# PJLab-ADG/OpenPCSeg

Hardware: AMD Instinct MI355X
Metric: LiDAR frames/sec training MinkUNet-34 SemanticKITTI (higher is better)
Workload: dtype f32; 1 GPU; MinkUNet-34 cr1.0 train step, 12 x 120k-pt synthetic SemanticKITTI scans/GPU, fp32; global_batch=12, voxels_per_gpu_batch=1158864, parallelism=dp1, wgrad=fp32

## Files before the change

include/pcseg_hip.h:

```cpp
#ifndef PCSEG_HIP_H_
#define PCSEG_HIP_H_

#include <stddef.h>
#include <stdint.h>

#ifdef __cplusplus
extern "C" {
#endif

#define PCS_OK 0
#define PCS_EINVAL (-1)
#define PCS_EWORKSPACE (-2)
#define PCS_ELAUNCH (-3)
#define PCS_EUNSUPPORTED (-4)

#define PCS_ABI_VERSION 12

int pcs_abi_version(void);
const char *pcs_last_error(void);

int pcs_hash(const int32_t *coords, int64_t n, int64_t *out, void *stream);

int pcs_kernel_hash(const int32_t *coords, int64_t n, const int32_t *offsets, int32_t K,
                    int64_t *out, void *stream);

int64_t pcs_hashtable_capacity(int64_t n);
size_t pcs_hashtable_bytes(int64_t capacity);
int pcs_hashtable_build(const int64_t *keys, int64_t n, void *table, int64_t capacity,
                        void *stream);
int pcs_hashtable_query(const void *table, int64_t capacity, const int64_t *queries,
                        int64_t n1, int64_t *out, void *stream);

int pcs_count(const int32_t *idx, int64_t n, int32_t *out, int64_t s, void *stream);

int pcs_voxelize_fwd_f32(const float *feats, const int32_t *idx, const int32_t *counts,
                         int64_t n, int64_t m, int32_t c, float *out, void *stream);
size_t pcs_index_csr_ws_bytes(int64_t n, int64_t m);
int pcs_index_csr_i32(const int32_t *index, int64_t n, int64_t m, int64_t *order, int64_t *rowptr, void *ws,
                      size_t ws_bytes, void *stream);
int pcs_voxelize_fwd_csr_f32(const float *feats, const int64_t *order, const int64_t *rowptr,
                             const int32_t *counts, int64_t m, int32_t c, float *out, void *stream);
int pcs_voxelize_bwd_f32(const float *gout, const int32_t *idx, const int32_t *counts,
                         int64_t n, int32_t c, float *gin, void *stream);

int pcs_devoxelize_fwd_f32(const float *feat, const int32_t *idx8, const float *w8, int64_t n,
                           int32_t c, float *out, void *stream);
int pcs_devoxelize_bwd_f32(const float *gout, const int32_t *idx8, const float *w8, int64_t n,
                           int64_t m, int32_t c, float *gfeat, void *stream);

int pcs_corner_map_f32(const float *coords, int32_t coord_ld, int64_t n, int32_t stride, const void *table,
                       int64_t capacity, int32_t *idx8, float *w8, void *stream);

int pcs_devoxelize_bwd_csr_f32(const float *gout, const int64_t *order, const int64_t *rowptr,
                               const float *w8, int64_t m, int32_t c, float *gfeat, void *stream);

int pcs_ti_weights_f32(const float *coords, int32_t coord_ld, const int64_t *idx_query,
                       int64_t n, float scale, float *w, void *stream);

int pcs_downsample_pack(const int32_t *coords, int64_t n, const int32_t *sample_stride3,
                        int32_t mode, const int32_t *offsets, int32_t K,
                        const int32_t *coords_min3, int64_t *keys, int32_t *err, void *stream);
int pcs_downsample_unpack(const int64_t *keys, int64_t m, int32_t *coords, void *stream);
size_t pcs_sort_unique_ws_bytes(int64_t n);
int pcs_sort_unique_i64(const int64_t *keys, int64_t n, int64_t *out, int64_t *info, const int32_t *err_flag, void *ws,
                        size_t ws_bytes, void *stream);

size_t pcs_rulebook_ws_bytes(int64_t nq, int32_t K);
int pcs_rulebook_probe(const int32_t *qcoords, int64_t nq, const int32_t *offsets, int32_t K,
                       const void *table, int64_t capacity, int32_t *results,
                       int64_t *nbsizes, void *ws, size_t ws_bytes, int32_t symmetric, void *stream);
int pcs_rulebook_fill(const int32_t *results, int64_t nq, int32_t K, const void *ws,
                      int32_t *pairs, int32_t *koff, void *stream);
int pcs_rulebook_tile_segments(const int32_t *pairs, const int32_t *koff, int32_t K,
                               int64_t n_dst, int32_t tile_rows, int32_t dst_col,
                               int32_t *seg, void *stream);
int pcs_rulebook_tile_order(const int32_t *seg, int32_t K, int64_t ntiles, int32_t *order, void *stream);

const char *pcs_conv_kernel_revision(void);
int32_t pcs_conv_tile_rows(int32_t cin, int32_t cout);
int32_t pcs_conv_pick_tile_rows(int64_t n_dst, int64_t n_pairs, int32_t K, int32_t cin, int32_t cout);
int32_t pcs_conv_pick_tile_rows_dt(int64_t n_dst, int64_t n_pairs, int32_t K, int32_t cin, int32_t cout,
                                   int32_t dtype);
int32_t pcs_conv_emits_bn_partials(int32_t cin, int32_t cout, int32_t K, int32_t tile_rows, int32_t dtype);
int32_t pcs_conv_uses_tile_order(int32_t cin, int32_t cout, int32_t K, int32_t dtype);
int pcs_conv_gather_gemm_f32(const float *src, int64_t n_src, int32_t cin, const float *W,
                             int32_t K, int32_t cout, const int32_t *pairs, int32_t src_col,
                             const int32_t *seg, int32_t tile_rows, int64_t n_dst,
                             const float *bias, float *dst, double *bn_partial, const int32_t *tile_order,
                             void *stream);
typedef struct pcs_conv_epilogue {
  const void *addend;
  float act_slope;
  int32_t reserved;
} pcs_conv_epilogue;
int pcs_conv_gather_gemm_f32_ex(const float *src, int64_t n_src, int32_t cin, const float *W,
                                int32_t K, int32_t cout, const int32_t *pairs, int32_t src_col,
                                const int32_t *seg, int32_t tile_rows, int64_t n_dst,
                                const float *bias, const pcs_conv_epilogue *ep, float *dst, double *bn_partial,
                                const int32_t *tile_order, void *stream);
int32_t pcs_conv_supports_epilogue(int32_t cin, int32_t cout, int32_t K, int32_t dtype);

int pcs_transpose_kab_f32(const float *src, int32_t K, int32_t A, int32_t B, float *dst, void *stream);

size_t pcs_conv_wgrad_ws_bytes(const int32_t *koff_host, int32_t K, int32_t ca, int32_t cb);
int pcs_conv_wgrad_f32(const float *fa, int32_t ca, const float *fb, int32_t cb,
                       const int32_t *pairs, int32_t a_col, const int32_t *koff_dev,
                       const int32_t *koff_host, int32_t K, float *gW, void *ws,
                       size_t ws_bytes, void *stream);

int pcs_scatter_max_fwd_f32(const float *src, const int64_t *order, const int64_t *rowptr, int64_t m,
                            int32_t c, float *out, int32_t *arg, void *stream);
int pcs_scatter_max_bwd_f32(const float *gout, const int32_t *arg, int64_t m, int64_t n, int32_t c,
                            float *gsrc, void *stream);

int pcs_map_count(const int32_t *pxpy, int64_t n, int32_t B, int32_t H, int32_t W, int32_t *out,
                  void *stream);
int pcs_denselize_fwd_f32(const float *feat, const int32_t *count_map, const int32_t *pxpy, int64_t n,
                          int32_t B, int32_t C, int32_t H, int32_t W, float *out, void *stream);
int pcs_denselize_fwd_csr_f32(const float *feat, const int64_t *order, const int64_t *rowptr,
                              const int32_t *count_map, int32_t B, int32_t C, int32_t H, int32_t W,
                              float *out, void *stream);
int pcs_denselize_bwd_csr_f32(const float *gout, const int64_t *order, const int64_t *rowptr,
                              const int32_t *count_map, int64_t n, int32_t B, int32_t C, int32_t H, int32_t W,
                              float *gfeat, void *stream);
int pcs_denselize_bwd_f32(const float *gout, const int32_t *count_map, const int32_t *pxpy, int64_t n,
                          int32_t B, int32_t C, int32_t H, int32_t W, float *gfeat, void *stream);

int pcs_range_sample_fwd_f32(const float *img, const float *pxpy, int64_t n, int32_t B, int32_t C, int32_t H, int32_t W,
                             float *out, void *stream);
int pcs_range_sample_corners(const float *pxpy, int64_t n, int32_t B, int32_t H, int32_t W, int64_t *keys, float *wts,
                             void *stream);
int pcs_range_sample_bwd_csr_f32(const float *gout, const int64_t *order, const int64_t *rowptr, const float *wts,
                                 int32_t B, int32_t C, int32_t H, int32_t W, float *gimg, void *stream);

int32_t pcs_bn_num_partials(void);
int pcs_bn_stats_f32(const float *x, int64_t n, int32_t c, float *partial_ws, double *sums, void *stream);
int pcs_bn_reduce_partials(const double *partial, int64_t nrows, int32_t c, int64_t n, double *sums, void *stream);
int pcs_bn_reduce_partials_finalize(const double *partial, int64_t nrows, int32_t c, int64_t n, double eps, double momentum,
                                    float *running_mean, float *running_var, double *sums, double *stat, void *stream);
int pcs_bn_finalize_f32(const double *sums, double count, const double *count_dev, int32_t c, double eps,
                        double momentum, float *running_mean, float *running_var, double *stat, void *stream);
int pcs_bn_apply_f32(const float *x, const float *res, const double *stat, const float *w, const float *b,
                     int64_t n, int32_t c, int32_t relu, float *y, uint32_t *mask, int64_t ldy, const float *tail,
                     int32_t ctail, void *stream);
int pcs_bn_bwd_stats_f32(const float *dy, const float *x, const float *y, const uint32_t *mask, const double *stat,
                         int64_t n, int32_t c, int32_t relu, float *partial_ws, double *sums2, int64_t sums2_doubles,
                         int64_t lddy, void *stream);
int pcs_bn_bwd_apply_f32(const float *dy, const float *x, const float *y, const uint32_t *mask, const double *stat,
                         const double *sums2, double count, const double *count_dev, const float *w, int64_t n,
                         int32_t c, int32_t relu, float *dx, float *dres, int64_t lddy, void *stream);
int pcs_bn_stats_h(const void *x, int64_t n, int32_t c, int32_t dtype, float *partial_ws, double *sums, void *stream);
int pcs_bn_apply_h(const void *x, const void *res, const double *stat, const float *w, const float *b, int64_t n,
                   int32_t c, int32_t relu, int32_t dtype, void *y, uint32_t *mask, int64_t ldy, const void *tail,
                   int32_t ctail, void *stream);
int pcs_bn_bwd_stats_h(const void *dy, const void *x, const void *y, const uint32_t *mask, const double *stat, int64_t n,
                       int32_t c, int32_t relu, int32_t dtype, float *partial_ws, double *sums2, int64_t sums2_doubles,
                       int64_t lddy, void *stream);
int pcs_bn_bwd_apply_h(const void *dy, const void *x, const void *y, const uint32_t *mask, const double *stat,
                       const double *sums2, double count, const double *count_dev, const float *w, int64_t n,
                       int32_t c, int32_t relu, int32_t dtype, void *dx, void *dres, int64_t lddy, void *stream);
int pcs_bn_bwd_apply_act(const void *dy, const void *x, const void *y, const uint32_t *mask, const double *stat,
                         const double *sums2, double count, const double *count_dev, const float *w, int64_t n, int32_t c,
                         int32_t relu, int32_t dtype, float in_slope, void *dx, void *dres, int64_t lddy, void *stream);

int pcs_quantize_floor(const void *points, int32_t is_float, int64_t n, int32_t row_stride,
                       const double *voxel_size3, int32_t *coords, int32_t *bbox, void *stream);
int pcs_quantize_keys(const int32_t *coords, int64_t n, const int32_t *bbox, int64_t *keys, void *stream);
int pcs_quantize_frame_keys(const int32_t *coords, const int64_t *frames, int64_t n, const int32_t *bbox, int64_t *keys, void *stream);
int pcs_quantize_flags(const int64_t *sorted_keys, int64_t n, int32_t *flags, void *stream);
int pcs_quantize_emit(const int32_t *flags, const int64_t *rank, const int64_t *perm, const int32_t *coords,
                      int64_t n, int32_t *vox, int64_t *index, int64_t *inverse, void *stream);

int pcs_unique_emit(const int32_t *flags, const int64_t *rank, const int64_t *perm, const int64_t *sorted_keys,
                    int64_t n, int64_t *uniq, int64_t *inverse, int64_t *rowptr, void *stream);

int pcs_conv_x3_applies(int32_t cin, int32_t cout, int32_t K);
int32_t pcs_conv_x3_column_tiles(int32_t cout);
int32_t pcs_conv_x3_emits_bn_partials(int32_t cin, int32_t cout, int32_t K, int32_t tile_rows);
size_t pcs_conv_prepared_weights_x3_bytes(int32_t K, int32_t ccon, int32_t ccols);
int pcs_conv_prepare_weights_x3(const float *W, int32_t K, int32_t A, int32_t B, int32_t transpose, void *Wp, void *stream);
int pcs_conv_gather_gemm_f32_bf16x3(const float *src, int64_t n_src, int32_t cin, const void *Wp, int32_t K, int32_t cout,
                                    const int32_t *pairs, int32_t src_col, const int32_t *seg, int32_t tile_rows,
                                    int64_t n_dst, const float *bias, float *dst, double *bn_partial,
// ... 54 lines not shown
```

openpcseg_amd/csrc/conv.hip:

```cpp
#include <math.h>

#include "conv_half.h"

using namespace pcs;

namespace pcs {
bool conv6h_applies(int cin, int cout, int K);
bool conv6h_is_chunked(int cin, int cout);
int conv6h_mode();
}

namespace {

int device_cus() {
  static int cus = 0;
  if (!cus) {
    int dev = 0, n = 0;
    if (hipGetDevice(&dev) == hipSuccess &&
        hipDeviceGetAttribute(&n, hipDeviceAttributeMultiprocessorCount, dev) == hipSuccess && n > 0) cus = n;
    else cus = 256;
  }
  return cus;
}

__global__ void __launch_bounds__(256) transpose_kab_kernel(const float *__restrict__ src, int A, int B,
                                                            float *__restrict__ dst) {
  __shared__ float tile[32][33];
  const int k = blockIdx.z, a0 = blockIdx.y * 32, b0 = blockIdx.x * 32;
  const int tx = threadIdx.x & 31, ty = threadIdx.x >> 5;
  const float *s = src + (int64_t)k * A * B;
  float *d = dst + (int64_t)k * A * B;
#pragma unroll
  for (int r = ty; r < 32; r += 8)
    if (a0 + r < A && b0 + tx < B) tile[r][tx] = s[(int64_t)(a0 + r) * B + b0 + tx];
  __syncthreads();
#pragma unroll
  for (int r = ty; r < 32; r += 8)
    if (b0 + r < B && a0 + tx < A) d[(int64_t)(b0 + r) * A + a0 + tx] = tile[tx][r];
}

}

extern "C" int pcs_transpose_kab_f32(const float *src, int32_t K, int32_t A, int32_t B, float *dst, void *stream) {
  if (K <= 0 || A <= 0 || B <= 0 || K > 65535 || !src || !dst) { set_error("pcs_transpose_kab_f32: bad args"); return PCS_EINVAL; }
  hipLaunchKernelGGL(transpose_kab_kernel, dim3((unsigned)ceil_div(B, 32), (unsigned)ceil_div(A, 32), (unsigned)K), dim3(256),
                     0, as_stream(stream), src, A, B, dst);
  return check_launch("pcs_transpose_kab_f32");
}

extern "C" const char *pcs_conv_kernel_revision(void) { return "r6.1"; }

extern "C" int32_t pcs_conv_tile_rows(int32_t cin, int32_t cout) {
  (void)cin;
  (void)cout;
  return 128;
}

namespace {
double launch_cost(int64_t n_dst, int T, int64_t ncol, double ppr, int K) {
  const double per_cu = (double)(ceil_div(n_dst, T) * ncol) / (double)device_cus();
  const double rounds = 0.5 * (ceil(per_cu) + per_cu);
  return rounds * (T * ppr + 8.0 * K);
}
}

extern "C" int32_t pcs_conv_pick_tile_rows_dt(int64_t n_dst, int64_t n_pairs, int32_t K, int32_t cin, int32_t cout,
                                              int32_t dtype) {
  static const int fixed = getenv("PCS_CONV_TILE") ? atoi(getenv("PCS_CONV_TILE")) : 0;
  if (n_dst <= 0 || K <= 0 || cin <= 0 || cout <= 0) return 128;
  if (!(dtype == 0 ? conv5_applies(cin, cout, K) : convh_applies(cin, cout, K))) return 128;
  if (fixed > 0) return fixed;
  const double ppr = (double)n_pairs / (double)n_dst;
  const int nctt = conv_nctt(cout);
  if (dtype != 0) {
    if (cin >= 256 && cout >= 256) {
      if (conv6h_mode() && conv6h_applies(cin, cout, K) && conv6h_is_chunked(cin, cout) && (cin > 256 || cout > 256 || n_dst <= 65536))
        return 144;
      const int64_t ncol = ceil_div(cout, 16 * nctt);
      return launch_cost(n_dst, 288, ncol, ppr, K) <= launch_cost(n_dst, 224, ncol, ppr, K) ? 288 : 224;
    }
    const int64_t ncol = ceil_div(cout, 16 * nctt);
    const int tmax = nctt == 6 ? 192 : 144;
    int best = tmax;
    double best_cost = launch_cost(n_dst, tmax, ncol, ppr, K);
    for (int T = tmax - 16; T >= tmax - 48; T -= 16) {
      const double c = launch_cost(n_dst, T, ncol, ppr, K);
      if (c < best_cost * 0.97) { best = T; best_cost = c; }
    }
    return best;
  }
  if (conv5_nctt(cout, 192) <= 4) {
    const int64_t ncol = ceil_div(cout, 16 * conv5_nctt(cout, 192));
    int best = 224;
    double best_cost = 0;
    for (int T = 192; T <= 288; T += 32) {
      const double c = launch_cost(n_dst, T, ncol, ppr, K);
      if (best_cost == 0 || c < best_cost) { best = T; best_cost = c; }
    }
    return best;
  }
  const int64_t ncol = ceil_div(cout, 16 * nctt);
  const int64_t slots = (int64_t)device_cus() * 2;
  if (ceil_div(n_dst, 128) * ncol >= 8 * slots && ppr < 6.5) {
    int T = 384;
    while (T > 128 && conv5_lds_est(T, nctt) > kMaxDynLds) T -= 32;
    if (T >= 192) return T;
  }
  int best = 128;
  double best_cost = launch_cost(n_dst, 128, ncol, ppr, K) * 0.97;
  for (int T = 80; T <= 192; T += 16) {
    if (T == 128) continue;
    if (2 * conv5_lds_est(T, nctt) > 160 * 1024) continue;
    const double c = launch_cost(n_dst, T, ncol, ppr, K);
    if (c < best_cost) { best = T; best_cost = c; }
  }
  return best;
}

extern "C" int32_t pcs_conv_pick_tile_rows(int64_t n_dst, int64_t n_pairs, int32_t K, int32_t cin, int32_t cout) {
  return pcs_conv_pick_tile_rows_dt(n_dst, n_pairs, K, cin, cout, 0);
}

extern "C" int32_t pcs_conv_emits_bn_partials(int32_t cin, int32_t cout, int32_t K, int32_t tile_rows, int32_t dtype) {
  if (cin <= 0 || cout <= 0 || K <= 0 || K > 32 || (cin % 4) || (cout % 4) || tile_rows < 16) return 0;
  int nctt = conv_nctt(cout), nt = 256;
  if (dtype == 0) {
    if (conv5_applies(cin, cout, K)) {
      nctt = conv5_nctt(cout, tile_rows);
      nt = 2 * conv5_lds_est(tile_rows, nctt) > 160 * 1024 ? 512 : 256;
    } else if (tile_rows != 64 && tile_rows != 128) {
      return 0;
    }
  } else {
// ... 69 lines not shown
```

openpcseg_amd/csrc/conv_common.h:

```cpp
#pragma once
#include <stdlib.h>

#include <type_traits>

#include "pcs_common.h"

#ifndef PCS_TRACE
#define PCS_TRACE 0
#endif
#ifndef PCS_ABLATE5
#define PCS_ABLATE5 0
#endif
#ifndef PCS_ABLATEH
#define PCS_ABLATEH 0
#endif
#ifndef PCS_ALIAS
#define PCS_ALIAS 0
#endif
#if PCS_TRACE
#define PCS_T(...) __VA_ARGS__
#else
#define PCS_T(...)
#endif

namespace pcs {

typedef float f32x4 __attribute__((ext_vector_type(4)));

struct ConvArgs {
  const float *src;
  const float *W;
  const float *bias;
  float *dst;
  const int32_t *pairs;
  const int32_t *seg;
  int64_t n_dst;
  int64_t ntiles;
  int cin, cout, K, src_col, ncoltiles, tile_rows;
  double *stats;
  const int32_t *order;
  const float *addend = nullptr;
  float act_slope = 1.f;
};

struct Bf16 {};
struct Fp16 {};
struct Fp32 {};
__device__ __forceinline__ float h2f(Bf16, uint16_t h) { return __uint_as_float((uint32_t)h << 16); }
__device__ __forceinline__ float h2f(Fp16, uint16_t h) { return (float)__builtin_bit_cast(_Float16, h); }
__device__ __forceinline__ uint16_t f2h(Bf16, float f) {
  uint32_t u = __float_as_uint(f);
  if ((u & 0x7FFFFFFFu) > 0x7F800000u) return (uint16_t)((u >> 16) | 0x40u);
  u += 0x7FFFu + ((u >> 16) & 1u);
  return (uint16_t)(u >> 16);
}
__device__ __forceinline__ uint16_t f2h(Fp16, float f) {
  const _Float16 h = (_Float16)f;
  return __builtin_bit_cast(uint16_t, h);
}

constexpr size_t kMaxDynLds = 160 * 1024 - 256;
constexpr int kConvSinkRows = 1;
inline size_t conv5_lds_est(int tile_rows, int nctt) { return (size_t)((tile_rows + kConvSinkRows) * (16 * nctt + 4)) * 4 + 1024; }

inline int conv_nctt(int cout) {
  int nctt = (cout + 15) / 16;
  if (nctt <= 8) {
    if (nctt == 5) nctt = 6;
    if (nctt == 7) nctt = 8;
    return nctt;
  }
  int best = 8, best_pad = ((cout + 127) / 128) * 128 - cout;
  for (int n = 6; n >= 4; n -= 2) {
    const int pad = ((cout + 16 * n - 1) / (16 * n)) * 16 * n - cout;
    if (pad < best_pad) { best = n; best_pad = pad; }
  }
  return best;
}
inline int conv5_nctt(int cout, int tile_rows) {
  if (cout >= 128 && cout % 64 == 0 && tile_rows >= 176) return 4;
  if (cout >= 192 && tile_rows >= 192) return 4;
  return conv_nctt(cout);
}
inline bool conv5_applies(int cin, int cout, int K) {
  return cin % 4 == 0 && cin >= 32 && cout % 4 == 0 && K <= 32 && conv_nctt(cout) % 2 == 0;
}

inline bool convh_applies(int cin, int cout, int K) {
  return cin % 8 == 0 && cin >= 32 && cout % 4 == 0 && K <= 32 && conv_nctt(cout) % 2 == 0;
}

template <int CT, int NT, typename Store>
__device__ __forceinline__ void conv_tile_epilogue(float *acc_l, int ACS, int rows, int n0, int cout, const float *bias,
                                                   double *stats, int tid, Store store) {
  constexpr int Q = CT / 4, NRG = NT / Q;
  const int q = tid % Q, rg = tid / Q, cq = 4 * q;
  const bool on = rg < NRG && n0 + cq < cout;
  float4 b = make_float4(0.f, 0.f, 0.f, 0.f), piv = b, s0 = b, s1 = b;
  if (on) {
    if (bias) b = *reinterpret_cast<const float4 *>(bias + n0 + cq);
    if (stats) {
      piv = *reinterpret_cast<const float4 *>(acc_l + cq);
      piv.x += b.x; piv.y += b.y; piv.z += b.z; piv.w += b.w;
    }
    for (int r = rg; r < rows; r += NRG) {
      float4 v = *reinterpret_cast<const float4 *>(acc_l + r * ACS + cq);
      v.x += b.x; v.y += b.y; v.z += b.z; v.w += b.w;
      const float4 sv = store(r, cq, v);
      if (stats) {
        const float dx = sv.x - piv.x, dy = sv.y - piv.y, dz = sv.z - piv.z, dw = sv.w - piv.w;
        s0.x += dx; s0.y += dy; s0.z += dz; s0.w += dw;
        s1.x += dx * dx; s1.y += dy * dy; s1.z += dz * dz; s1.w += dw * dw;
      }
    }
  }
  if (stats) {
    __syncthreads();
    if (on) {
      *reinterpret_cast<float4 *>(acc_l + (2 * rg) * ACS + cq) = s0;
      *reinterpret_cast<float4 *>(acc_l + (2 * rg + 1) * ACS + cq) = s1;
      if (rg == 0) *reinterpret_cast<float4 *>(acc_l + (2 * NRG) * ACS + cq) = piv;
    }
    __syncthreads();
    if (tid < CT && n0 + tid < cout) {
      double t0 = 0.0, t1 = 0.0;
      for (int h = 0; h < NRG; ++h) { t0 += (double)acc_l[(2 * h) * ACS + tid]; t1 += (double)acc_l[(2 * h + 1) * ACS + tid]; }
      const double p = (double)acc_l[(2 * NRG) * ACS + tid], dn = (double)rows;
      stats[n0 + tid] = t0 + dn * p;
      stats[cout + n0 + tid] = t1 + 2.0 * p * t0 + dn * p * p;
    }
  }
}
inline bool conv_stats_fit(int tile_rows, int ct, int nt) { return tile_rows + 1 >= 2 * (nt / (ct / 4)) + 1; }

int launch_conv_block(ConvArgs a, bool vec, hipStream_t st);
int launch_conv_wave4(ConvArgs a, hipStream_t st);
int launch_conv_wave5(ConvArgs a, hipStream_t st);

}
```

openpcseg_amd/csrc/conv_wave5.hip:

```cpp
#include "conv_common.h"

using namespace pcs;

namespace {

#if PCS_TRACE
__device__ long long *g_conv_trace;
constexpr int kTraceBlocks = 8192;
#endif

template <int NCTT, int NW_, int R_>
struct Conv5Cfg {
  static constexpr int NW = NW_;
  static constexpr int R = R_;
  static constexpr int NT = 64 * NW;
  static constexpr int CT = 16 * NCTT;
  static constexpr int ACS = CT + 4;
  static constexpr int N4 = NCTT / 4;
  static constexpr int N2 = (NCTT % 4) / 2;
  static constexpr int N1 = NCTT % 2;
  static constexpr int NWL = N4 + N2 + N1;
  static constexpr int SINK = kConvSinkRows;
  static constexpr size_t lds_bytes(int T) { return (size_t)((T + SINK) * ACS) * 4 + 5 * 33 * 4 + 16; }
};

template <int NCTT, int NW, int MINW, int R, bool TAIL>
__global__ void __launch_bounds__(64 * NW, MINW) conv_os5_kernel(ConvArgs a) {
  using C = Conv5Cfg<NCTT, NW, R>;
  const int T = a.tile_rows;
  PCS_T(const long long tr_entry = wall_clock64(); long long tr_loop = 0, tr_ticket = 0, tr_commit = 0; int tr_groups = 0;)
  extern __shared__ __attribute__((aligned(16))) char smem[];
  float *acc_l = reinterpret_cast<float *>(smem);
  int *kl_k = reinterpret_cast<int *>(acc_l + (T + C::SINK) * C::ACS);
  int *kl_s = kl_k + 32;
  int *kl_m = kl_s + 32;
  int *kl_g = kl_m + 32;
  int *kl_h = kl_g + 33;
  int *commit = kl_h + 33;
  const unsigned commit_lds = (unsigned)(size_t)(__attribute__((address_space(3))) int *)commit;
  const unsigned acc_lds = (unsigned)(size_t)(__attribute__((address_space(3))) float *)acc_l;
  __shared__ int nk_s;

  const int tid = threadIdx.x, lane = tid & 63, wid = __builtin_amdgcn_readfirstlane(tid >> 6);
  const int g = lane >> 4, l15 = lane & 15;
  unsigned bid = blockIdx.x;
  if (!a.order) {
    const unsigned nb = gridDim.x, q = nb >> 3, r = nb & 7, xcd = bid & 7, idx = bid >> 3;
    bid = (xcd < r ? xcd * (q + 1) : r * (q + 1) + (xcd - r) * q) + idx;
  }
  int64_t slot = bid / a.ncoltiles;
  int ctile = bid % a.ncoltiles;
  if (a.order) {
    const unsigned xcd = bid & 7, idx = bid >> 3;
    slot = (int64_t)(idx / a.ncoltiles) * 8 + xcd;
    ctile = idx % a.ncoltiles;
    if (slot >= a.ntiles) return;
  }
  const int64_t tile = a.order ? (int64_t)a.order[slot] : slot;
  const int n0 = ctile * C::CT;
  const int64_t row0 = tile * T;
  const int64_t nt1 = a.ntiles + 1;

  if (wid == 0) {
    const int k = lane;
    int s0 = 0, m = 0;
    if (k < a.K) {
      s0 = a.seg[(int64_t)k * nt1 + tile];
      m = a.seg[(int64_t)k * nt1 + tile + 1] - s0;
    }
    const unsigned long long mask = __ballot(m > 0);
    const int nrb = (m + 15) >> 4;
    const int nfull = nrb / R, npart = (nrb % R) ? 1 : 0;
    int incl = nfull | (npart << 16);
    for (int o = 1; o < 64; o <<= 1) {
      const int t = __shfl_up(incl, o, 64);
      if (lane >= o) incl += t;
    }
    if (m > 0) {
      const int pos = __popcll(mask & ((1ULL << lane) - 1ULL));
      kl_k[pos] = k; kl_s[pos] = s0; kl_m[pos] = m;
      kl_g[pos] = (incl & 0xFFFF) - nfull; kl_h[pos] = (incl >> 16) - npart;
    }
    const int total = __shfl(incl, 63, 64);
    if (lane == 0) {
      const int nkk = __popcll(mask);
      nk_s = nkk; kl_g[nkk] = total & 0xFFFF; kl_h[nkk] = total >> 16; *commit = 0;
    }
  }
  {
    float4 *z = reinterpret_cast<float4 *>(acc_l);
    const int n4 = (T + C::SINK) * (C::ACS / 4);
    for (int i = tid; i < n4; i += C::NT) z[i] = make_float4(0.f, 0.f, 0.f, 0.f);
  }
  __syncthreads();
  const int nk = __builtin_amdgcn_readfirstlane(nk_s);
  const int total_full = nk > 0 ? __builtin_amdgcn_readfirstlane(kl_g[nk]) : 0;
  const int total_grp = nk > 0 ? total_full + __builtin_amdgcn_readfirstlane(kl_h[nk]) : 0;

  const int cin4 = a.cin - 4;
  const int nb16 = TAIL ? (a.cin + 15) >> 4 : a.cin >> 4;
  const int cinp = nb16 * 16;
  int col4[C::N4 > 0 ? C::N4 : 1];
#pragma unroll
  for (int q = 0; q < C::N4; ++q) {
    const int c = 64 * q + 4 * l15;
    col4[q] = (n0 + c + 4 <= a.cout) ? c : 0;
  }
  const int c2 = 64 * C::N4 + 2 * l15;
  const int col2 = (n0 + c2 + 2 <= a.cout) ? c2 : 0;
  const int c1 = 64 * C::N4 + 32 * C::N2 + l15;
  const int col1 = (n0 + c1 < a.cout) ? c1 : 0;

  struct Frag {
    float4 a[R];
    float4 b4[4][C::N4 > 0 ? C::N4 : 1];
    float2 b2[4];
    float b1[4];
  };
  struct Ctx {
    const float *srow0[R];
    const float *Wk;
    int dloc[R];
    int nr;
    unsigned vmask;
  };
  auto load_frag = [&](Frag &f, const Ctx &cx, int c0, bool in_loop = false) {
    int ca = c0 + 4 * g;
    if (TAIL) ca = ca < cin4 ? ca : cin4;
    (void)in_loop;
#if PCS_ABLATE5 == 3
    if (in_loop) return;
#endif
#if PCS_ABLATE5 != 6
#pragma unroll
    for (int r = 0; r < R; ++r) f.a[r] = *reinterpret_cast<const float4 *>(cx.srow0[r] + ca);
#else
    if (!in_loop) for (int r = 0; r < R; ++r) f.a[r] = *reinterpret_cast<const float4 *>(cx.srow0[r] + ca);
#endif
#if PCS_ABLATE5 == 5
    if (in_loop) return;
#endif
// ... 164 lines not shown
#pragma unroll
    for (int r = 0; r < R; ++r)
#pragma unroll
      for (int j = 0; j < 4; ++j) {
        dq[r][j] = acc_lds + 4u * (unsigned)doff[r][j] + 16u * l15;
        dp[r][j] = acc_lds + 4u * (unsigned)doff[r][j] + 256u * C::N4 + (C::N2 ? 8u : 4u) * l15;
        asm volatile("" : "+v"(dq[r][j]), "+v"(dp[r][j]));
      }
    if (lane == 0) {
      while (__hip_atomic_load(commit, __ATOMIC_RELAXED, __HIP_MEMORY_SCOPE_WORKGROUP) != grp)
        __builtin_amdgcn_s_sleep(1);
    }
    __builtin_amdgcn_fence(__ATOMIC_ACQUIRE, "workgroup", "local");
    __builtin_amdgcn_s_setprio(3);
    PCS_T(const long long tr_c = wall_clock64();)
    {
      typedef float v2f __attribute__((ext_vector_type(2)));
      typedef __attribute__((address_space(3))) const f32x4 lds_cf4;
      typedef __attribute__((address_space(3))) const v2f lds_cf2;
      typedef __attribute__((address_space(3))) const float lds_cf1;
      typedef __attribute__((address_space(3))) f32x4 lds_f4;
      typedef __attribute__((address_space(3))) v2f lds_f2;
      typedef __attribute__((address_space(3))) float lds_f1;
      constexpr int RB = (NCTT <= 6) ? NRC : 1;
#pragma unroll
      for (int r0 = 0; r0 < NRC; r0 += RB) {
        f32x4 v4[RB][4][C::N4 > 0 ? C::N4 : 1];
        v2f v2[RB][4];
        float v1[RB][4];
#pragma unroll
        for (int rr = 0; rr < RB; ++rr)
#pragma unroll
          for (int j = 0; j < 4; ++j) {
            const int r = r0 + rr;
#pragma unroll
            for (int q = 0; q < C::N4; ++q) v4[rr][j][q] = *(lds_cf4 *)(size_t)(dq[r][j] + 256u * q);
            if (C::N2) v2[rr][j] = *(lds_cf2 *)(size_t)dp[r][j];
            if (C::N1) v1[rr][j] = *(lds_cf1 *)(size_t)(dp[r][j] + 128u * C::N2);
          }
        asm volatile("" ::: "memory");
#pragma unroll
        for (int rr = 0; rr < RB; ++rr)
#pragma unroll
          for (int j = 0; j < 4; ++j) {
            const int r = r0 + rr;
#pragma unroll
            for (int q = 0; q < C::N4; ++q) {
              v4[rr][j][q].x += acc[r][4 * q + 0][j]; v4[rr][j][q].y += acc[r][4 * q + 1][j];
              v4[rr][j][q].z += acc[r][4 * q + 2][j]; v4[rr][j][q].w += acc[r][4 * q + 3][j];
            }
            if (C::N2) { v2[rr][j].x += acc[r][4 * C::N4 + 0][j]; v2[rr][j].y += acc[r][4 * C::N4 + 1][j]; }
            if (C::N1) v1[rr][j] += acc[r][NCTT - 1][j];
          }
        asm volatile("" ::: "memory");
#pragma unroll
        for (int rr = 0; rr < RB; ++rr)
#pragma unroll
          for (int j = 0; j < 4; ++j) {
            const int r = r0 + rr;
#pragma unroll
            for (int q = 0; q < C::N4; ++q) *(lds_f4 *)(size_t)(dq[r][j] + 256u * q) = v4[rr][j][q];
            if (C::N2) *(lds_f2 *)(size_t)dp[r][j] = v2[rr][j];
            if (C::N1) *(lds_f1 *)(size_t)(dp[r][j] + 128u * C::N2) = v1[rr][j];
          }
        asm volatile("" ::: "memory");
      }
    }
    if (lane == 0) asm volatile("ds_write_b32 %0, %1" ::"v"(commit_lds), "v"(grp + 1) : "memory");
    __builtin_amdgcn_s_setprio(0);
    PCS_T(const long long tr_d = wall_clock64(); tr_loop += tr_b - tr_a; tr_ticket += tr_c - tr_b; tr_commit += tr_d - tr_c; ++tr_groups;)
    cur = nxt;
    i = in;
  };
  {
    int grp = wid;
    for (; grp < total_full; grp += C::NW) run_group(grp, std::integral_constant<int, R>{});
    for (; grp < total_grp; grp += C::NW) run_group(grp, std::integral_constant<int, 1>{});
  }
  PCS_T(const long long tr_end = wall_clock64();)
  __syncthreads();
  const int rows = (int)((a.n_dst - row0) < (int64_t)T ? (a.n_dst - row0) : (int64_t)T);
  float *drow = a.dst + row0 * a.cout + n0;
  const int ldd = a.cout;
  conv_tile_epilogue<C::CT, C::NT>(acc_l, C::ACS, rows, n0, a.cout, a.bias, a.stats ? a.stats + tile * 2 * a.cout : nullptr, tid,
                                   [&](int r, int cq, const float4 &v0) {
                                     float4 v = v0;
                                     if (a.addend) {
                                       const float4 ad = *reinterpret_cast<const float4 *>(a.addend + (row0 + r) * (int64_t)ldd + n0 + cq);
                                       v.x += ad.x; v.y += ad.y; v.z += ad.z; v.w += ad.w;
                                     }
                                     if (a.act_slope != 1.f) {
                                       v.x = v.x < 0.f ? v.x * a.act_slope : v.x; v.y = v.y < 0.f ? v.y * a.act_slope : v.y;
                                       v.z = v.z < 0.f ? v.z * a.act_slope : v.z; v.w = v.w < 0.f ? v.w * a.act_slope : v.w;
                                     }
                                     *reinterpret_cast<float4 *>(drow + (int64_t)r * ldd + cq) = v;
                                     return v;
                                   });
#if PCS_TRACE
  if (lane == 0 && blockIdx.x < kTraceBlocks && g_conv_trace) {
    long long *t = g_conv_trace + ((int64_t)blockIdx.x * 8 + wid) * 8;
    t[0] = tr_entry; t[1] = tr_start; t[2] = tr_end; t[3] = tr_loop; t[4] = tr_ticket; t[5] = tr_commit;
    t[6] = tr_groups; t[7] = wall_clock64();
  }
#endif
}

#if PCS_TRACE
long long *g_trace_host_ptr = nullptr;
void trace_prepare(hipStream_t st) {
  if (!g_trace_host_ptr) {
    (void)hipMalloc(&g_trace_host_ptr, (size_t)kTraceBlocks * 64 * sizeof(long long));
    (void)hipMemcpyToSymbol(HIP_SYMBOL(g_conv_trace), &g_trace_host_ptr, sizeof(g_trace_host_ptr));
  }
  (void)hipMemsetAsync(g_trace_host_ptr, 0, (size_t)kTraceBlocks * 64 * sizeof(long long), st);
}
#endif

template <int NCTT, int NW, int MINW, int R, bool TAIL>
int launch_conv5(const ConvArgs &a, hipStream_t st) {
  using C = Conv5Cfg<NCTT, NW, R>;
  const int64_t nblocks = a.order ? ceil_div(a.ntiles, 8) * 8 * a.ncoltiles : a.ntiles * a.ncoltiles;
  if (nblocks <= 0) return PCS_OK;
  if (nblocks > 0x7FFFFFFF) { set_error("pcs_conv: grid too large"); return PCS_EUNSUPPORTED; }
  auto kern = conv_os5_kernel<NCTT, NW, MINW, R, TAIL>;
  const size_t lds = C::lds_bytes(a.tile_rows);
  if (lds > kMaxDynLds) { set_error("pcs_conv: tile_rows too large for this column tile"); return PCS_EUNSUPPORTED; }
  static bool attr_set = false;
  if (!attr_set) {
    (void)hipFuncSetAttribute(reinterpret_cast<const void *>(kern),
                              hipFuncAttributeMaxDynamicSharedMemorySize, (int)kMaxDynLds);
    attr_set = true;
  }
  PCS_T(trace_prepare(st);)
  static const int dbg = getenv("PCS_CONV_DEBUG") ? atoi(getenv("PCS_CONV_DEBUG")) : 0;
  static long long dbg_last = -1;
  const long long dbg_key = ((long long)a.tile_rows << 32) ^ ((long long)a.cin << 16) ^ a.cout;
  if (dbg && dbg_key != dbg_last) {
    dbg_last = dbg_key;
    int nb = 0;
    (void)hipOccupancyMaxActiveBlocksPerMultiprocessor(&nb, reinterpret_cast<const void *>(kern), C::NT, lds);
    fprintf(stderr, "[pcs_conv] wave5<%d,%d,%d,%d%s> T=%d cin=%d cout=%d grid=%lld lds=%zu resident WG/CU=%d (waves/SIMD=%d)\n", NCTT, NW,
            MINW, R, TAIL ? ",tail" : "", a.tile_rows, a.cin, a.cout, (long long)nblocks, lds, nb, nb * NW / 4);
  }
  hipLaunchKernelGGL(kern, dim3((unsigned)nblocks), dim3(C::NT), lds, st, a);
  return check_launch("pcs_conv_gather_gemm_f32(wave5)");
}

}

#if PCS_TRACE
extern "C" int pcs_debug_conv_trace(long long *host_out) {
  if (!g_trace_host_ptr || !host_out) return PCS_EINVAL;
  if (hipDeviceSynchronize() != hipSuccess) return PCS_ELAUNCH;
  return hipMemcpy(host_out, g_trace_host_ptr, (size_t)kTraceBlocks * 64 * sizeof(long long), hipMemcpyDeviceToHost) == hipSuccess ? PCS_OK : PCS_ELAUNCH;
}
#endif

int pcs::launch_conv_wave5(ConvArgs a, hipStream_t st) {
  int nctt = conv5_nctt(a.cout, a.tile_rows);
  static const int force_nctt = getenv("PCS_CONV_NCTT") ? atoi(getenv("PCS_CONV_NCTT")) : 0;
  static const int force_nw = getenv("PCS_CONV_NW") ? atoi(getenv("PCS_CONV_NW")) : 0;
  if (force_nctt && nctt > force_nctt) nctt = force_nctt;
  a.ncoltiles = (int)ceil_div(a.cout, 16 * nctt);
  const bool nw8 = force_nw ? force_nw == 8 : 2 * conv5_lds_est(a.tile_rows, nctt) > 160 * 1024;
  const bool tail = (a.cin % 32) != 0;
#define PCS_CONV5_CASE(N)                                                                           \
  case N:                                                                                           \
    if (nw8) return tail ? launch_conv5<N, 8, 2, 2, true>(a, st) : launch_conv5<N, 8, 2, 2, false>(a, st);  \
    return tail ? launch_conv5<N, 4, 2, 2, true>(a, st) : launch_conv5<N, 4, 2, 2, false>(a, st);
  switch (nctt) {
    PCS_CONV5_CASE(2)
    PCS_CONV5_CASE(4)
    PCS_CONV5_CASE(6)
    PCS_CONV5_CASE(8)
  }
#undef PCS_CONV5_CASE
  set_error("pcs_conv_gather_gemm_f32: unreachable");
  return PCS_EINVAL;
}
```

openpcseg_amd/native.py:

```python
import ctypes
import os
from ctypes import c_char_p, c_double, c_float, c_int32, c_int64, c_size_t, c_void_p

import torch

_LIB_PATH = os.environ.get("PCS_LIB_PATH") or os.path.join(os.path.dirname(os.path.abspath(__file__)), "lib",
                                                          "libpcseg_hip.so")

_P = c_void_p
SIGNATURES = {
    "pcs_abi_version": (c_int32, []),
    "pcs_last_error": (c_char_p, []),
    "pcs_hash": (c_int32, [_P, c_int64, _P, _P]),
    "pcs_kernel_hash": (c_int32, [_P, c_int64, _P, c_int32, _P, _P]),
    "pcs_hashtable_capacity": (c_int64, [c_int64]),
    "pcs_hashtable_bytes": (c_size_t, [c_int64]),
    "pcs_hashtable_build": (c_int32, [_P, c_int64, _P, c_int64, _P]),
    "pcs_hashtable_query": (c_int32, [_P, c_int64, _P, c_int64, _P, _P]),
    "pcs_count": (c_int32, [_P, c_int64, _P, c_int64, _P]),
    "pcs_voxelize_fwd_f32": (c_int32, [_P, _P, _P, c_int64, c_int64, c_int32, _P, _P]),
    "pcs_voxelize_fwd_csr_f32": (c_int32, [_P, _P, _P, _P, c_int64, c_int32, _P, _P]),
    "pcs_voxelize_bwd_f32": (c_int32, [_P, _P, _P, c_int64, c_int32, _P, _P]),
    "pcs_devoxelize_fwd_f32": (c_int32, [_P, _P, _P, c_int64, c_int32, _P, _P]),
    "pcs_devoxelize_bwd_f32": (c_int32, [_P, _P, _P, c_int64, c_int64, c_int32, _P, _P]),
    "pcs_devoxelize_bwd_csr_f32": (c_int32, [_P, _P, _P, _P, c_int64, c_int32, _P, _P]),
    "pcs_corner_map_f32": (c_int32, [_P, c_int32, c_int64, c_int32, _P, c_int64, _P, _P, _P]),
    "pcs_ti_weights_f32": (c_int32, [_P, c_int32, _P, c_int64, c_float, _P, _P]),
    "pcs_downsample_pack": (c_int32, [_P, c_int64, _P, c_int32, _P, c_int32, _P, _P, _P, _P]),
    "pcs_downsample_unpack": (c_int32, [_P, c_int64, _P, _P]),
    "pcs_index_csr_ws_bytes": (c_size_t, [c_int64, c_int64]),
    "pcs_index_csr_i32": (c_int32, [_P, c_int64, c_int64, _P, _P, _P, c_size_t, _P]),
    "pcs_sort_unique_ws_bytes": (c_size_t, [c_int64]),
    "pcs_sort_unique_i64": (c_int32, [_P, c_int64, _P, _P, _P, _P, c_size_t, _P]),
    "pcs_rulebook_ws_bytes": (c_size_t, [c_int64, c_int32]),
    "pcs_rulebook_probe": (c_int32, [_P, c_int64, _P, c_int32, _P, c_int64, _P, _P, _P, c_size_t, c_int32, _P]),
    "pcs_rulebook_fill": (c_int32, [_P, c_int64, c_int32, _P, _P, _P, _P]),
    "pcs_rulebook_tile_segments": (c_int32, [_P, _P, c_int32, c_int64, c_int32, c_int32, _P, _P]),
    "pcs_rulebook_tile_order": (c_int32, [_P, c_int32, c_int64, _P, _P]),
    "pcs_conv_kernel_revision": (c_char_p, []),
    "pcs_conv_tile_rows": (c_int32, [c_int32, c_int32]),
    "pcs_conv_pick_tile_rows": (c_int32, [c_int64, c_int64, c_int32, c_int32, c_int32]),
    "pcs_conv_pick_tile_rows_dt": (c_int32, [c_int64, c_int64, c_int32, c_int32, c_int32, c_int32]),
    "pcs_conv_emits_bn_partials": (c_int32, [c_int32, c_int32, c_int32, c_int32, c_int32]),
    "pcs_conv_uses_tile_order": (c_int32, [c_int32, c_int32, c_int32, c_int32]),
    "pcs_conv_gather_gemm_f32": (c_int32, [_P, c_int64, c_int32, _P, c_int32, c_int32, _P, c_int32,
                                           _P, c_int32, c_int64, _P, _P, _P, _P, _P]),
    "pcs_conv_gather_gemm_f32_ex": (c_int32, [_P, c_int64, c_int32, _P, c_int32, c_int32, _P, c_int32,
                                              _P, c_int32, c_int64, _P, _P, _P, _P, _P, _P]),
    "pcs_conv_supports_epilogue": (c_int32, [c_int32, c_int32, c_int32, c_int32]),
    "pcs_bn_bwd_apply_act": (c_int32, [_P, _P, _P, _P, _P, _P, c_double, _P, _P, c_int64, c_int32, c_int32, c_int32, c_float, _P, _P,
                                       c_int64, _P]),
    "pcs_bn_reduce_partials": (c_int32, [_P, c_int64, c_int32, c_int64, _P, _P]),
    "pcs_bn_reduce_partials_finalize": (c_int32, [_P, c_int64, c_int32, c_int64, c_double, c_double, _P, _P, _P, _P, _P]),
    "pcs_transpose_kab_f32": (c_int32, [_P, c_int32, c_int32, c_int32, _P, _P]),
    "pcs_conv_wgrad_ws_bytes": (c_size_t, [_P, c_int32, c_int32, c_int32]),
    "pcs_conv_wgrad_f32": (c_int32, [_P, c_int32, _P, c_int32, _P, c_int32, _P, _P, c_int32, _P,
                                     _P, c_size_t, _P]),
    "pcs_scatter_max_fwd_f32": (c_int32, [_P, _P, _P, c_int64, c_int32, _P, _P, _P]),
    "pcs_scatter_max_bwd_f32": (c_int32, [_P, _P, c_int64, c_int64, c_int32, _P, _P]),
    "pcs_map_count": (c_int32, [_P, c_int64, c_int32, c_int32, c_int32, _P, _P]),
    "pcs_denselize_fwd_f32": (c_int32, [_P, _P, _P, c_int64, c_int32, c_int32, c_int32, c_int32, _P, _P]),
    "pcs_denselize_fwd_csr_f32": (c_int32, [_P, _P, _P, _P, c_int32, c_int32, c_int32, c_int32, _P, _P]),
    "pcs_denselize_bwd_csr_f32": (c_int32, [_P, _P, _P, _P, c_int64, c_int32, c_int32, c_int32, c_int32, _P, _P]),
    "pcs_denselize_bwd_f32": (c_int32, [_P, _P, _P, c_int64, c_int32, c_int32, c_int32, c_int32, _P, _P]),
    "pcs_range_sample_fwd_f32": (c_int32, [_P, _P, c_int64, c_int32, c_int32, c_int32, c_int32, _P, _P]),
    "pcs_range_sample_corners": (c_int32, [_P, c_int64, c_int32, c_int32, c_int32, _P, _P, _P]),
    "pcs_range_sample_bwd_csr_f32": (c_int32, [_P, _P, _P, _P, c_int32, c_int32, c_int32, c_int32, _P, _P]),
    "pcs_bn_num_partials": (c_int32, []),
    "pcs_bn_stats_f32": (c_int32, [_P, c_int64, c_int32, _P, _P, _P]),
    "pcs_bn_finalize_f32": (c_int32, [_P, c_double, _P, c_int32, c_double, c_double, _P, _P, _P, _P]),
    "pcs_bn_apply_f32": (c_int32, [_P, _P, _P, _P, _P, c_int64, c_int32, c_int32, _P, _P, c_int64, _P, c_int32, _P]),
    "pcs_bn_bwd_stats_f32": (c_int32, [_P, _P, _P, _P, _P, c_int64, c_int32, c_int32, _P, _P, c_int64, c_int64, _P]),
    "pcs_bn_bwd_apply_f32": (c_int32, [_P, _P, _P, _P, _P, _P, c_double, _P, _P, c_int64, c_int32, c_int32, _P, _P,
                                       c_int64, _P]),
    "pcs_bn_stats_h": (c_int32, [_P, c_int64, c_int32, c_int32, _P, _P, _P]),
    "pcs_bn_apply_h": (c_int32, [_P, _P, _P, _P, _P, c_int64, c_int32, c_int32, c_int32, _P, _P, c_int64, _P, c_int32, _P]),
    "pcs_bn_bwd_stats_h": (c_int32, [_P, _P, _P, _P, _P, c_int64, c_int32, c_int32, c_int32, _P, _P, c_int64, c_int64, _P]),
    "pcs_bn_bwd_apply_h": (c_int32, [_P, _P, _P, _P, _P, _P, c_double, _P, _P, c_int64, c_int32, c_int32, c_int32, _P, _P,
                                     c_int64, _P]),
    "pcs_quantize_floor": (c_int32, [_P, c_int32, c_int64, c_int32, _P, _P, _P, _P]),
    "pcs_quantize_keys": (c_int32, [_P, c_int64, _P, _P, _P]),
    "pcs_quantize_frame_keys": (c_int32, [_P, _P, c_int64, _P, _P, _P]),
    "pcs_quantize_flags": (c_int32, [_P, c_int64, _P, _P]),
    "pcs_quantize_emit": (c_int32, [_P, _P, _P, _P, c_int64, _P, _P, _P, _P]),
    "pcs_conv_h_applies": (c_int32, [c_int32, c_int32, c_int32]),
    "pcs_conv_prepared_weights_bytes": (c_size_t, [c_int32, c_int32, c_int32]),
    "pcs_conv_prepare_weights_h": (c_int32, [_P, c_int32, c_int32, c_int32, c_int32, c_int32, _P, _P]),
    "pcs_conv_gather_gemm_h": (c_int32, [_P, c_int64, c_int32, _P, c_int32, c_int32, _P, c_int32, _P, c_int32, c_int64,
                                         _P, _P, c_int32, _P, _P, _P]),
    "pcs_conv_gather_gemm_h_ex": (c_int32, [_P, c_int64, c_int32, _P, c_int32, c_int32, _P, c_int32, _P, c_int32, c_int64,
                                            _P, _P, _P, c_int32, _P, _P, _P]),
    "pcs_conv_x3_applies": (c_int32, [c_int32, c_int32, c_int32]),
    "pcs_conv_x3_column_tiles": (c_int32, [c_int32]),
    "pcs_conv_x3_emits_bn_partials": (c_int32, [c_int32, c_int32, c_int32, c_int32]),
    "pcs_conv_prepared_weights_x3_bytes": (c_size_t, [c_int32, c_int32, c_int32]),
    "pcs_conv_prepare_weights_x3": (c_int32, [_P, c_int32, c_int32, c_int32, c_int32, _P, _P]),
    "pcs_conv_gather_gemm_f32_bf16x3": (c_int32, [_P, c_int64, c_int32, _P, c_int32, c_int32, _P, c_int32, _P, c_int32, c_int64,
                                                  _P, _P, _P, _P, _P]),
    "pcs_conv_wgrad_f32_bf16x3": (c_int32, [_P, c_int32, _P, c_int32, _P, c_int32, _P, _P, c_int32, _P,
                                            _P, c_size_t, _P]),
    "pcs_conv_wgrad_h": (c_int32, [_P, c_int32, _P, c_int32, _P, c_int32, _P, _P, c_int32, _P, _P, c_size_t, c_int32, _P]),
    "pcs_unique_emit": (c_int32, [_P, _P, _P, _P, c_int64, _P, _P, _P, _P]),
    "pcs_cylinder_partition_f32": (c_int32, [_P, c_int64, c_int32, _P, _P, _P, _P, _P, _P, _P]),
    "pcs_voxel_label_vote": (c_int32, [_P, _P, c_int64, c_int64, c_int32, c_int64, _P, _P, _P, _P]),
    "pcs_rows_argmax_gather_f32": (c_int32, [_P, c_int64, c_int32, _P, c_int64, _P, _P]),
    "pcs_weights_multi_plan": (c_int64, [_P, c_int32]),
    "pcs_weights_multi": (c_int32, [_P, c_int32, c_int64, _P]),
    "pcs_lovasz_workspace_bytes": (c_int64, [c_int64, c_int32, c_int32, c_int64]),
    "pcs_lovasz_softmax_f32": (c_int32, [_P, _P, c_int64, c_int32, c_int32, c_int64, _P, _P, _P, c_int64, _P]),
    "pcs_debug_convh_ws": (None, [c_int32, c_int32, c_int32]),
    "pcs_debug_wgrad_interleave": (None, [c_int32]),
}

class _WeightJob(ctypes.Structure):
    _fields_ = [("src", c_void_p), ("dst", c_void_p), ("K", c_int32), ("A", c_int32), ("B", c_int32), ("kind", c_int32),
                ("transpose", c_int32), ("nctt", c_int32), ("nt16", c_int32), ("ns", c_int32), ("first_block", c_int64)]


ABI_VERSION = 12
_lib = None


def lib_path():
    return _LIB_PATH


def load_library():
    global _lib
    if _lib is not None:
        return _lib
    if not os.path.exists(_LIB_PATH):
        raise RuntimeError(
# ... 1006 lines not shown
```

Baseline: 105.6 frames/s.

## Taper conv tail wave by splitting final row tiles into narrower column tiles

```diff
diff --git a/include/pcseg_hip.h b/include/pcseg_hip.h
--- a/include/pcseg_hip.h
+++ b/include/pcseg_hip.h
@@ -99,6 +99,10 @@
                                 const float *bias, const pcs_conv_epilogue *ep, float *dst, double *bn_partial,
                                 const int32_t *tile_order, void *stream);
 int32_t pcs_conv_supports_epilogue(int32_t cin, int32_t cout, int32_t K, int32_t dtype);
+
+int32_t pcs_conv_set_tail_taper(int32_t n);
+int64_t pcs_conv_tail_taper_auto(int64_t ntiles, int32_t ncoltiles, int64_t slots, int32_t half_rounds);
+int64_t pcs_conv_tail_taper_map(int64_t ntiles, int32_t ncoltiles, int64_t n_narrow, int32_t *units, int64_t cap);
 
 int pcs_transpose_kab_f32(const float *src, int32_t K, int32_t A, int32_t B, float *dst, void *stream);
 
diff --git a/openpcseg_amd/csrc/conv.hip b/openpcseg_amd/csrc/conv.hip
--- a/openpcseg_amd/csrc/conv.hip
+++ b/openpcseg_amd/csrc/conv.hip
@@ -10,9 +10,7 @@
 int conv6h_mode();
 }
 
-namespace {
-
-int device_cus() {
+int pcs::device_cus() {
   static int cus = 0;
   if (!cus) {
     int dev = 0, n = 0;
@@ -22,6 +20,8 @@
   }
   return cus;
 }
+
+namespace {
 
 __global__ void __launch_bounds__(256) transpose_kab_kernel(const float *__restrict__ src, int A, int B,
                                                             float *__restrict__ dst) {
@@ -48,7 +48,7 @@
   return check_launch("pcs_transpose_kab_f32");
 }
 
-extern "C" const char *pcs_conv_kernel_revision(void) { return "r6.1"; }
+extern "C" const char *pcs_conv_kernel_revision(void) { return "r7.0"; }
 
 extern "C" int32_t pcs_conv_tile_rows(int32_t cin, int32_t cout) {
   (void)cin;
diff --git a/openpcseg_amd/csrc/conv_common.h b/openpcseg_amd/csrc/conv_common.h
--- a/openpcseg_amd/csrc/conv_common.h
+++ b/openpcseg_amd/csrc/conv_common.h
@@ -41,7 +41,39 @@
   const int32_t *order;
   const float *addend = nullptr;
   float act_slope = 1.f;
+  int64_t n_wide = 0;
 };
+
+constexpr int kConvTaperHalfRounds = 2;
+inline int64_t conv_taper_auto(int64_t ntiles, int ncol, int64_t slots, int half_rounds) {
+  const int64_t units = ntiles * ncol;
+  if (units <= slots || half_rounds < 0) return 0;
+  const int64_t tail_units = units % slots + slots * half_rounds / 2;
+  int64_t n_narrow = (tail_units + ncol - 1) / ncol;
+  if (n_narrow > ntiles / 2) n_narrow = ntiles / 2;
+  const int64_t n_wide = ((ntiles - n_narrow + 7) / 8) * 8;
+  return n_wide >= ntiles ? 0 : ntiles - n_wide;
+}
+struct ConvUnit {
+  int64_t slot;
+  int ctile;
+  int narrow;
+};
+__host__ __device__ inline int64_t conv_taper_grid(int64_t ntiles, int ncol, int64_t n_wide) {
+  return ((n_wide + 7) / 8) * 8 * ncol + ((ntiles - n_wide + 7) / 8) * 8 * 2 * ncol;
+}
+__host__ __device__ inline ConvUnit conv_taper_unit(int64_t bid, int64_t ntiles, int ncol, int64_t n_wide) {
+  const int64_t wide_blocks = ((n_wide + 7) / 8) * 8 * ncol;
+  ConvUnit u;
+  u.narrow = bid >= wide_blocks ? 1 : 0;
+  const int64_t b = u.narrow ? bid - wide_blocks : bid;
+  const int nc = u.narrow ? 2 * ncol : ncol;
+  const int64_t xcd = b & 7, idx = b >> 3;
+  const int64_t s = (idx / nc) * 8 + xcd;
+  u.ctile = (int)(idx % nc);
+  u.slot = u.narrow ? (n_wide + s < ntiles ? n_wide + s : -1) : (s < n_wide ? s : -1);
+  return u;
+}
 
 struct Bf16 {};
 struct Fp16 {};
@@ -90,10 +122,11 @@
   return cin % 8 == 0 && cin >= 32 && cout % 4 == 0 && K <= 32 && conv_nctt(cout) % 2 == 0;
 }
 
-template <int CT, int NT, typename Store>
+template <int CT, int NT, int NRGP = 0, typename Store>
 __device__ __forceinline__ void conv_tile_epilogue(float *acc_l, int ACS, int rows, int n0, int cout, const float *bias,
                                                    double *stats, int tid, Store store) {
-  constexpr int Q = CT / 4, NRG = NT / Q;
+  constexpr int Q = CT / 4, NRG = NRGP ? NRGP : NT / Q;
+  static_assert(NRG * Q <= NT, "more row groups than threads");
   const int q = tid % Q, rg = tid / Q, cq = 4 * q;
   const bool on = rg < NRG && n0 + cq < cout;
   float4 b = make_float4(0.f, 0.f, 0.f, 0.f), piv = b, s0 = b, s1 = b;
@@ -133,6 +166,8 @@
 }
 inline bool conv_stats_fit(int tile_rows, int ct, int nt) { return tile_rows + 1 >= 2 * (nt / (ct / 4)) + 1; }
 
+int device_cus();
+
 int launch_conv_block(ConvArgs a, bool vec, hipStream_t st);
 int launch_conv_wave4(ConvArgs a, hipStream_t st);
 int launch_conv_wave5(ConvArgs a, hipStream_t st);
diff --git a/openpcseg_amd/csrc/conv_wave5.hip b/openpcseg_amd/csrc/conv_wave5.hip
--- a/openpcseg_amd/csrc/conv_wave5.hip
+++ b/openpcseg_amd/csrc/conv_wave5.hip
@@ -1,3 +1,5 @@
+#include <atomic>
+
 #include "conv_common.h"
 
 using namespace pcs;
@@ -24,8 +26,8 @@
   static constexpr size_t lds_bytes(int T) { return (size_t)((T + SINK) * ACS) * 4 + 5 * 33 * 4 + 16; }
 };
 
-template <int NCTT, int NW, int MINW, int R, bool TAIL>
-__global__ void __launch_bounds__(64 * NW, MINW) conv_os5_kernel(ConvArgs a) {
+template <int NCTT, int NW, int R, bool TAIL, int NRGP>
+__device__ __forceinline__ void conv5_tile(const ConvArgs &a, const int64_t tile, const int ctile) {
   using C = Conv5Cfg<NCTT, NW, R>;
   const int T = a.tile_rows;
   PCS_T(const long long tr_entry = wall_clock64(); long long tr_loop = 0, tr_ticket = 0, tr_commit = 0; int tr_groups = 0;)
@@ -43,20 +45,6 @@
 
   const int tid = threadIdx.x, lane = tid & 63, wid = __builtin_amdgcn_readfirstlane(tid >> 6);
   const int g = lane >> 4, l15 = lane & 15;
-  unsigned bid = blockIdx.x;
-  if (!a.order) {
-    const unsigned nb = gridDim.x, q = nb >> 3, r = nb & 7, xcd = bid & 7, idx = bid >> 3;
-    bid = (xcd < r ? xcd * (q + 1) : r * (q + 1) + (xcd - r) * q) + idx;
-  }
-  int64_t slot = bid / a.ncoltiles;
-  int ctile = bid % a.ncoltiles;
-  if (a.order) {
-    const unsigned xcd = bid & 7, idx = bid >> 3;
-    slot = (int64_t)(idx / a.ncoltiles) * 8 + xcd;
-    ctile = idx % a.ncoltiles;
-    if (slot >= a.ntiles) return;
-  }
-  const int64_t tile = a.order ? (int64_t)a.order[slot] : slot;
   const int n0 = ctile * C::CT;
   const int64_t row0 = tile * T;
   const int64_t nt1 = a.ntiles + 1;
@@ -387,7 +375,7 @@
   const int rows = (int)((a.n_dst - row0) < (int64_t)T ? (a.n_dst - row0) : (int64_t)T);
   float *drow = a.dst + row0 * a.cout + n0;
   const int ldd = a.cout;
-  conv_tile_epilogue<C::CT, C::NT>(acc_l, C::ACS, rows, n0, a.cout, a.bias, a.stats ? a.stats + tile * 2 * a.cout : nullptr, tid,
+  conv_tile_epilogue<C::CT, C::NT, NRGP>(acc_l, C::ACS, rows, n0, a.cout, a.bias, a.stats ? a.stats + tile * 2 * a.cout : nullptr, tid,
                                    [&](int r, int cq, const float4 &v0) {
                                      float4 v = v0;
                                      if (a.addend) {
@@ -410,6 +398,38 @@
 #endif
 }
 
+template <int NCTT, int NW, int MINW, int R, bool TAIL>
+__global__ void __launch_bounds__(64 * NW, MINW) conv_os5_kernel(ConvArgs a) {
+  unsigned bid = blockIdx.x;
+  if (!a.order) {
+    const unsigned nb = gridDim.x, q = nb >> 3, r = nb & 7, xcd = bid & 7, idx = bid >> 3;
+    bid = (xcd < r ? xcd * (q + 1) : r * (q + 1) + (xcd - r) * q) + idx;
+  }
+  int64_t slot = bid / a.ncoltiles;
+  int ctile = bid % a.ncoltiles;
+  if (a.order) {
+    const unsigned xcd = bid & 7, idx = bid >> 3;
+    slot = (int64_t)(idx / a.ncoltiles) * 8 + xcd;
+    ctile = idx % a.ncoltiles;
+    if (slot >= a.ntiles) return;
+  }
+  const int64_t tile = a.order ? (int64_t)a.order[slot] : slot;
+  conv5_tile<NCTT, NW, R, TAIL, 0>(a, tile, ctile);
+}
+
+template <int NCW, int NCN, int NW, int MINW, int R, bool TAIL>
+__global__ void __launch_bounds__(64 * NW, MINW) conv_os5_taper_kernel(ConvArgs a) {
+  const ConvUnit u = conv_taper_unit(blockIdx.x, a.ntiles, a.ncoltiles, a.n_wide);
+  if (u.slot < 0) return;
+  const int64_t tile = a.order[u.slot];
+  if (!u.narrow) {
+    conv5_tile<NCW, NW, R, TAIL, 0>(a, tile, u.ctile);
+  } else {
+    if (u.ctile * 16 * NCN >= a.cout) return;
+    conv5_tile<NCN, NW, R, TAIL, 16 * NW / NCW>(a, tile, u.ctile);
+  }
+}
+
 #if PCS_TRACE
 long long *g_trace_host_ptr = nullptr;
 void trace_prepare(hipStream_t st) {
@@ -451,6 +471,61 @@
   return check_launch("pcs_conv_gather_gemm_f32(wave5)");
 }
 
+constexpr int kNoTaper = 1;
+std::atomic<int> g_tail_taper{-1};
+
+template <int NCW, int NCN, int NW, int MINW, int R, bool TAIL>
+int launch_conv5_taper(ConvArgs &a, hipStream_t st) {
+  using C = Conv5Cfg<NCW, NW, R>;
+  auto kern = conv_os5_taper_kernel<NCW, NCN, NW, MINW, R, TAIL>;
+  const size_t lds = C::lds_bytes(a.tile_rows);
+  if (lds > kMaxDynLds || a.ntiles <= 0) return kNoTaper;
+  static bool attr_set = false;
+  if (!attr_set) {
+    (void)hipFuncSetAttribute(reinterpret_cast<const void *>(kern),
+                              hipFuncAttributeMaxDynamicSharedMemorySize, (int)kMaxDynLds);
+    attr_set = true;
+  }
+  const int mode = g_tail_taper.load(std::memory_order_relaxed);
+  int64_t n_narrow = mode;
+  if (mode < 0) {
+    static int per_cu[33] = {};
+    int &nb = per_cu[a.tile_rows / 16];
+    if (!nb) {
+      if (hipOccupancyMaxActiveBlocksPerMultiprocessor(&nb, reinterpret_cast<const void *>(kern), C::NT, lds) != hipSuccess || nb <= 0) nb = 1;
+    }
+    n_narrow = conv_taper_auto(a.ntiles, a.ncoltiles, (int64_t)device_cus() * nb, kConvTaperHalfRounds);
+  }
+  if (n_narrow > a.ntiles) n_narrow = a.ntiles;
+  if (n_narrow <= 0) return kNoTaper;
+  a.n_wide = a.ntiles - n_narrow;
+  const int64_t nblocks = conv_taper_grid(a.ntiles, a.ncoltiles, a.n_wide);
+  if (nblocks > 0x7FFFFFFF) { set_error("pcs_conv: grid too large"); return PCS_EUNSUPPORTED; }
+  PCS_T(trace_prepare(st);)
+  hipLaunchKernelGGL(kern, dim3((unsigned)nblocks), dim3(C::NT), lds, st, a);
+  return check_launch("pcs_conv_gather_gemm_f32(wave5 taper)");
+}
+
+}
+
+extern "C" int32_t pcs_conv_set_tail_taper(int32_t n) { return g_tail_taper.exchange(n < -1 ? -1 : n); }
+
+extern "C" int64_t pcs_conv_tail_taper_auto(int64_t ntiles, int32_t ncoltiles, int64_t slots, int32_t half_rounds) {
+  if (ntiles <= 0 || ncoltiles <= 0 || slots <= 0) return 0;
+  return conv_taper_auto(ntiles, ncoltiles, slots, half_rounds < 0 ? kConvTaperHalfRounds : half_rounds);
+}
+
+extern "C" int64_t pcs_conv_tail_taper_map(int64_t ntiles, int32_t ncoltiles, int64_t n_narrow, int32_t *units, int64_t cap) {
+  if (ntiles <= 0 || ncoltiles <= 0) return 0;
+  n_narrow = n_narrow < 0 ? 0 : (n_narrow > ntiles ? ntiles : n_narrow);
+  const int64_t n_wide = ntiles - n_narrow, grid = conv_taper_grid(ntiles, ncoltiles, n_wide);
+  for (int64_t b = 0; units && b < grid && b < cap; ++b) {
+    const ConvUnit u = conv_taper_unit(b, ntiles, ncoltiles, n_wide);
+    units[3 * b + 0] = (int32_t)u.slot;
+    units[3 * b + 1] = u.narrow ? 2 * u.ctile : 4 * u.ctile;
+    units[3 * b + 2] = u.slot < 0 ? 0 : (u.narrow ? 2 : 4);
+  }
+  return grid;
 }
 
 #if PCS_TRACE
@@ -469,7 +544,12 @@
   a.ncoltiles = (int)ceil_div(a.cout, 16 * nctt);
   const bool nw8 = force_nw ? force_nw == 8 : 2 * conv5_lds_est(a.tile_rows, nctt) > 160 * 1024;
   const bool tail = (a.cin % 32) != 0;
-#define PCS_CONV5_CASE(N)                                                                           \
+  if (a.order && nctt == 4 && g_tail_taper.load(std::memory_order_relaxed) != 0) {
+    const int rc = nw8 ? (tail ? launch_conv5_taper<4, 2, 8, 2, 2, true>(a, st) : launch_conv5_taper<4, 2, 8, 2, 2, false>(a, st))
+                       : (tail ? launch_conv5_taper<4, 2, 4, 2, 2, true>(a, st) : launch_conv5_taper<4, 2, 4, 2, 2, false>(a, st));
+    if (rc != kNoTaper) return rc;
+  }
+#define PCS_CONV5_CASE(N)                                                                          \
   case N:                                                                                           \
     if (nw8) return tail ? launch_conv5<N, 8, 2, 2, true>(a, st) : launch_conv5<N, 8, 2, 2, false>(a, st);  \
     return tail ? launch_conv5<N, 4, 2, 2, true>(a, st) : launch_conv5<N, 4, 2, 2, false>(a, st);
diff --git a/openpcseg_amd/native.py b/openpcseg_amd/native.py
--- a/openpcseg_amd/native.py
+++ b/openpcseg_amd/native.py
@@ -48,6 +48,9 @@
     "pcs_conv_gather_gemm_f32_ex": (c_int32, [_P, c_int64, c_int32, _P, c_int32, c_int32, _P, c_int32,
                                               _P, c_int32, c_int64, _P, _P, _P, _P, _P, _P]),
     "pcs_conv_supports_epilogue": (c_int32, [c_int32, c_int32, c_int32, c_int32]),
+    "pcs_conv_set_tail_taper": (c_int32, [c_int32]),
+    "pcs_conv_tail_taper_auto": (c_int64, [c_int64, c_int32, c_int64, c_int32]),
+    "pcs_conv_tail_taper_map": (c_int64, [c_int64, c_int32, c_int64, _P, c_int64]),
     "pcs_bn_bwd_apply_act": (c_int32, [_P, _P, _P, _P, _P, _P, c_double, _P, _P, c_int64, c_int32, c_int32, c_int32, c_float, _P, _P,
                                        c_int64, _P]),
     "pcs_bn_reduce_partials": (c_int32, [_P, c_int64, c_int32, c_int64, _P, _P]),
```

New measurement: 103.5 frames/s. -2.0%, worse.
